# shanjiayao/PTT

Measured on AMD Instinct MI355X. Metric: tracklet frames/sec (hot path: PointNet++ SA stack + Point-Track-Transformer blocks), higher is better.
Workload: dtype f32

## Files before the change

### include/ptt_hip.h

```cpp
#ifndef PTT_HIP_H
#define PTT_HIP_H

#include <stddef.h>
#include <stdint.h>

#ifdef __cplusplus
extern "C" {
#endif

#define PTT_ABI_VERSION 25

enum {
    PTT_OK = 0,
    PTT_EINVAL = -1,
    PTT_EUNSUPPORTED = -2,
    PTT_ELAUNCH = -3,
    PTT_EWORKSPACE = -4
};

typedef void* ptt_stream_t;

int ptt_version(void);
const char* ptt_error_name(int code);
const char* ptt_last_error_string(void);

int ptt_fps_f32(const float* xyz, int B, int N, int npoint, int32_t* idx_out,
                ptt_stream_t stream);
int ptt_fps_ws_f32(const float* xyz, int B, int N, int npoint, int32_t* idx_out, float* workspace,
                   size_t workspace_elems, ptt_stream_t stream);

int ptt_gather_f32(const float* feat, const int32_t* idx, int B, int C, int N, int M,
                   float* out, ptt_stream_t stream);
int ptt_gather_grad_f32(const float* grad_out, const int32_t* idx, int B, int C, int N,
// ... 447 lines not shown
```

### ptt_amd/_lib.py

```python
import ctypes
import os
from ctypes import POINTER, Structure, c_char_p, c_double, c_float, c_int, c_int32, c_int64, c_longlong, c_size_t, c_uint32, c_void_p

_HERE = os.path.dirname(os.path.abspath(__file__))
LIB_PATH = os.path.join(_HERE, "lib", "libptt_hip.so")

PTT_SA_MAX_LAYERS = 4
ABI_VERSION = 25

EXPORTS = [
    "ptt_version", "ptt_error_name", "ptt_last_error_string",
    "ptt_fps_f32", "ptt_fps_ws_f32", "ptt_spatial_order_f32", "ptt_ball_query_grid_workspace", "ptt_ball_query_grid_f32",
    "ptt_centres_ball_query_grid_f32", "ptt_gather_f32", "ptt_gather_grad_f32", "ptt_select_centres_f32", "ptt_ball_query_f32",
    "ptt_group_f32", "ptt_group_grad_f32", "ptt_scatter_add_det_workspace", "ptt_scatter_add_det_f32",
    "ptt_knn_f32", "ptt_knn_rel_f32",
    "ptt_packed_weight_elems", "ptt_pack_weight_f32", "ptt_pack_weight_rot_f32", "ptt_linear_f32",
    "ptt_sa_fused_fwd_f32", "ptt_xcorr_fused_fwd_f32", "ptt_cosine_map_f32", "ptt_pt_attn_pair_f32",
    "ptt_crop_compact_f32", "ptt_regularize_f32", "ptt_mt19937_fill", "ptt_select_box_f32",
    "ptt_track_crop_bounds", "ptt_track_box_by_offset",
    "ptt_bn_stats_workspace", "ptt_bn_stats_f32", "ptt_bn_apply_f32", "ptt_bn_bwd_f32", "ptt_pool_rows_f32",
    "ptt_pool_rows_bwd_f32", "ptt_linear_wgrad_workspace", "ptt_linear_wgrad_f32",
    "ptt_pack_weight_strided_f32", "ptt_linear_batched_f32", "ptt_softmax_rows_f32", "ptt_layernorm_f32",
    "ptt_gather_rows_f32", "ptt_scatter_csr_i32", "ptt_scatter_rows_csr_f32",
    "ptt_pt_pair_input_f32", "ptt_pt_attn_train_fwd_f32", "ptt_pt_attn_train_bwd_f32", "ptt_linear_act_in_f32",
    "ptt_centres_ball_query_f32",
    "ptt_bn_sums_f64", "ptt_bn_finish_f64", "ptt_bn_bwd_sums_f64", "ptt_bn_bwd_apply_f32",
    "ptt_rows_mlp_f32",
    "ptt_rows_gemm_supported", "ptt_rows_gemm_stat_chunks", "ptt_rows_gemm_f32", "ptt_rows_gemm_masked_f32", "ptt_bn_finish_partials_f32",
    "ptt_bn_sums_partials_f64", "ptt_linear_wgrad2_workspace", "ptt_linear_wgrad2_f32",
    "ptt_bn_bwd_pooled_f32", "ptt_bn_bwd_pooled_sums_f64", "ptt_bn_bwd_pooled_apply_f32",
    "ptt_pt_pair_input_ld_f32", "ptt_pt_attn_fwd_ld_f32",
# ... 302 lines not shown
```

### ptt_amd/csrc/mfma_ops.hip

```cpp
#include <math.h>
#include <stdlib.h>
#include <string.h>
#include "common.h"
#include "mfma_common.h"

#ifndef PTT_PAIR_PF
#define PTT_PAIR_PF 1
#endif
#ifndef PTT_GATHER_BATCH
#define PTT_GATHER_BATCH 16
#endif
#ifndef PTT_SA_WAVES
#define PTT_SA_WAVES 2
#endif

namespace ptt {

#ifdef PTT_DEV
#define PTT_STAMP(i) do { if (p.dbg && threadIdx.x == 0 && blockIdx.x < 4096) p.dbg[blockIdx.x * 8 + (i)] = __builtin_readcyclecounter(); } while (0)
#else
#define PTT_STAMP(i) do { } while (0)
#endif

__device__ __forceinline__ void stagger_second_slot(int first_wave_blocks, int quanta) {
// ... 1243 lines not shown
                        p.out[b * p.osb + col * p.osc + mm * p.osm] = m1;
                    }
                }
            }
        }
    }
    __builtin_amdgcn_wave_barrier();
}

constexpr int SAC_HDR = 16;
struct SacTable {
    int32_t* ws; int T;
    __host__ __device__ int32_t* ndist() const { return ws + SAC_HDR; }
    __host__ __device__ int32_t* list(int k) const { return ws + SAC_HDR + (size_t)(1 + k) * T; }
    __host__ __device__ int32_t* rows(int k) const { return ws + SAC_HDR + 5 * (size_t)T + (size_t)((4 << k) - 4) * T; }
    static size_t words(size_t T) { return SAC_HDR + 65 * T; }
};
constexpr int SAC_PASSES = 4;

__global__ __launch_bounds__(64) void sa_compact_zero_kernel(int32_t* ws) {
    if (threadIdx.x < 4) ws[threadIdx.x] = 0;
}

__global__ __launch_bounds__(256) void sa_compact_kernel(const float* __restrict__ xyz, const int32_t* __restrict__ idx, int N, int M,
                                                         SacTable tab) {
    __shared__ int s_cnt[4], s_base[4], s_cls[32], s_pos[32], s_nd[32];
    __shared__ int s_row[32][32];
    const int t = threadIdx.x, lane = t & 63, half = lane >> 5, s = lane & 31, w = t >> 6;
    const int g0 = blockIdx.x * 32, T = tab.T;
    if (t < 4) s_cnt[t] = 0;
    __syncthreads();
    int iv[SAC_PASSES];
    uint32_t x[SAC_PASSES], y[SAC_PASSES], z[SAC_PASSES];
#pragma unroll
    for (int q = 0; q < SAC_PASSES; ++q) iv[q] = idx[(size_t)min(g0 + q * 8 + w * 2 + half, T - 1) * 32 + s];
#pragma unroll
    for (int q = 0; q < SAC_PASSES; ++q) {
        const int b = min(g0 + q * 8 + w * 2 + half, T - 1) / M;
        const uint32_t* pt = reinterpret_cast<const uint32_t*>(xyz) + ((size_t)b * N + iv[q]) * 3;
        x[q] = pt[0]; y[q] = pt[1]; z[q] = pt[2];
    }
#pragma unroll
    for (int q = 0; q < SAC_PASSES; ++q) {
        const int lc = q * 8 + w * 2 + half;
        const int i0a = __builtin_amdgcn_readlane(iv[q], 0), i0b = __builtin_amdgcn_readlane(iv[q], 32);
        const int i0 = half ? i0b : i0a;
        const bool real = s == 0 || iv[q] != i0;
        const unsigned long long rm = __ballot(real);
        const int J = 31 - __builtin_clz((uint32_t)rm | (uint32_t)(rm >> 32));
        int dup = 0;
        for (int j = 0; j < J; ++j) {
            const uint32_t xa = __builtin_amdgcn_readlane(x[q], j), xb = __builtin_amdgcn_readlane(x[q], 32 + j);
            const uint32_t ya = __builtin_amdgcn_readlane(y[q], j), yb = __builtin_amdgcn_readlane(y[q], 32 + j);
            const uint32_t za = __builtin_amdgcn_readlane(z[q], j), zb = __builtin_amdgcn_readlane(z[q], 32 + j);
            dup |= (int)(j < s) & (int)(x[q] == (half ? xb : xa)) & (int)(y[q] == (half ? yb : ya)) & (int)(z[q] == (half ? zb : za));
        }
        const bool keep = real && !dup;
        const unsigned long long km = __ballot(keep);
        const uint32_t m = half ? (uint32_t)(km >> 32) : (uint32_t)km;
        const int nd = __popc(m);
        if (keep) s_row[lc][__popc(m & ((1u << s) - 1u))] = iv[q];
        if (s == 0) {
            const int k = nd <= 4 ? 0 : nd <= 8 ? 1 : nd <= 16 ? 2 : 3;
            const bool valid = g0 + lc < T;
            s_cls[lc] = valid ? k : -1;
            s_nd[lc] = nd;
            s_pos[lc] = valid ? atomicAdd(&s_cnt[k], 1) : 0;
            if (valid) tab.ndist()[g0 + lc] = nd;
        }
    }
    __syncthreads();
    if (t < 4) s_base[t] = s_cnt[t] ? atomicAdd(&tab.ws[t], s_cnt[t]) : 0;
    __syncthreads();
    for (int e = t; e < 32 * 32; e += 256) {
        const int lc = e >> 5, j = e & 31, k = s_cls[lc];
        if (k < 0 || j >= (4 << k)) continue;
        const int q = s_base[k] + s_pos[lc];
        tab.rows(k)[(size_t)q * (4 << k) + j] = s_row[lc][j < s_nd[lc] ? j : 0];
        if (j == 0) tab.list(k)[q] = g0 + lc;
    }
}

#ifndef PTT_SAL_WGS
#define PTT_SAL_WGS 1
#endif
#ifndef PTT_SAL_WAVES
#define PTT_SAL_WAVES 12
#endif

struct SacTile {
    int k, first, n;
    __device__ __forceinline__ void at(int j, const int (&tiles)[4], const int (&cnt)[4]) {
        k = j < tiles[0] ? 0 : j < tiles[1] ? 1 : j < tiles[2] ? 2 : 3;
        const int j0 = k == 0 ? 0 : k == 1 ? tiles[0] : k == 2 ? tiles[1] : tiles[2];
        const int nk = k == 0 ? cnt[0] : k == 1 ? cnt[1] : k == 2 ? cnt[2] : cnt[3];
        first = (j - j0) << (3 - k);
        n = min(8 >> k, nk - first);
    }
    __device__ __forceinline__ void row(const SacTable& tab, int s, int& n_out, int& ball) const {
        const int cl = s >> (2 + k), inb = cl < n;
        n_out = tab.rows(k)[(size_t)first * (4 << k) + (inb ? s : (s & ((4 << k) - 1)))];
        ball = tab.list(k)[first + (inb ? cl : 0)];
    }
};

__device__ __forceinline__ void sac_store(const SaParams& p, const SacTile& tc, int ball, const f32x16 (&acc)[4], const float* cst,
                                          int half, int col, int osb, int osm, int osc) {
    const int k = tc.k, relu = p.L[2].relu;
    int ob[8];
#pragma unroll
    for (int g = 0; g < 8; ++g) {
        if (g >= (8 >> k)) break;
        const int id = __builtin_amdgcn_readlane(ball, g << (2 + k)), b = id / p.M;
        ob[g] = b * osb + (id - b * p.M) * osm;
    }
#pragma unroll
    for (int u = 0; u < 4; ++u) {
        const float sh = cst[(6 + u) * 64];
        float* o = p.out + (u * 32 + col) * osc;
        const f32x16& a = acc[u];
        if (k == 3) {
            const float mx = sas_pool(a, sh, relu);
            if (half == 0) o[ob[0]] = mx;
        } else if (k == 2) {
            float m0 = a[0], m1 = a[8];
#pragma unroll
            for (int r = 1; r < 8; ++r) { m0 = fmaxf(m0, a[r]); m1 = fmaxf(m1, a[8 + r]); }
            m0 = max_halves(m0) + sh; m1 = max_halves(m1) + sh;
            if (relu) { m0 = fmaxf(m0, 0.f); m1 = fmaxf(m1, 0.f); }
            if (half < tc.n) o[half ? ob[1] : ob[0]] = half ? m1 : m0;
        } else {
            float m[4];
#pragma unroll
            for (int q = 0; q < 4; ++q) m[q] = fmaxf(fmaxf(a[4 * q], a[4 * q + 1]), fmaxf(a[4 * q + 2], a[4 * q + 3]));
            if (k == 1) {
#pragma unroll
                for (int q = 0; q < 4; ++q) m[q] = max_halves(m[q]) + sh;
#pragma unroll
                for (int i = 0; i < 2; ++i) {
                    const int g = 2 * half + i;
                    float v = half ? m[2 + i] : m[i];
                    if (relu) v = fmaxf(v, 0.f);
                    if (g < tc.n) o[half ? ob[2 + i] : ob[i]] = v;
                }
            } else {
#pragma unroll
                for (int q = 0; q < 4; ++q) {
                    const int g = 2 * q + half;
                    float v = m[q] + sh;
                    if (relu) v = fmaxf(v, 0.f);
                    if (g < tc.n) o[half ? ob[2 * q + 1] : ob[2 * q]] = v;
                }
            }
        }
    }
}

template <bool COMPACT>
__global__ __launch_bounds__(64 * PTT_SAL_WAVES) __attribute__((amdgpu_waves_per_eu(PTT_SAL_WAVES * PTT_SAL_WGS / 4)))
void sa_lds_kernel(SaParams p) {
    extern __shared__ __attribute__((aligned(16))) float smem[];
    float* W1 = smem;
    float* W2 = smem + 4096;
    const int t = threadIdx.x, lane = t & 63, half = lane >> 5, col = lane & 31;
    const int w = __builtin_amdgcn_readfirstlane(t >> 6);
    const int total = p.B * p.M, M = p.M, N = p.N;
    const int nw = (int)blockDim.x >> 6;
    SacTable tab{p.cws, total};
    int cnt[4], tiles[4];
    if constexpr (COMPACT) {
#pragma unroll
        for (int k = 0; k < 4; ++k) {
            cnt[k] = min(max(p.cws[k], 0), total);
            tiles[k] = (k ? tiles[k - 1] : 0) + ((cnt[k] + (8 >> k) - 1) >> (3 - k));
        }
        if (logical_block() >= tiles[3]) return;
    }
    {
        const f32x4* g1 = reinterpret_cast<const f32x4*>(p.L[1].Wp);
        const f32x4* g2 = reinterpret_cast<const f32x4*>(p.L[2].Wp);
        f32x4* s1 = reinterpret_cast<f32x4*>(W1);
        f32x4* s2 = reinterpret_cast<f32x4*>(W2);
        const int nthr = (int)blockDim.x;
        for (int i = t; i < 1024; i += nthr) s1[i] = g1[i];
        for (int i = t; i < 2048; i += nthr) s2[i] = g2[i];
    }
    float* cst = smem + 4096 + 8192 + w * 640 + lane;
#pragma unroll
    for (int u = 0; u < 2; ++u) {
        const f32x4 f = reinterpret_cast<const f32x4*>(p.L[0].Wp)[u * 64 + col];
        const float s0 = p.L[0].shift ? p.L[0].shift[u * 32 + col] : 0.f;
        cst[(0 + u) * 64] = half ? f[1] : f[0];
        cst[(2 + u) * 64] = half ? s0 : f[2];
        cst[(4 + u) * 64] = p.L[1].shift ? p.L[1].shift[u * 32 + col] : 0.f;
    }
#pragma unroll
    for (int u = 0; u < 4; ++u) cst[(6 + u) * 64] = p.L[2].shift ? p.L[2].shift[u * 32 + col] : 0.f;
    const float one_zero = half ? 0.f : 1.f, one_hi = 1.f;
// ... 97 lines not shown
            cx = p.new_xyz[(size_t)g * 3]; cy = p.new_xyz[(size_t)g * 3 + 1]; cz = p.new_xyz[(size_t)g * 3 + 2];
        }
        __builtin_amdgcn_sched_barrier(0);
        {
            f32x16 acc[4];
#pragma unroll
            for (int kb = 0; kb < 8; ++kb) {
                if (kb < 7) {
#pragma unroll
                    for (int u = 0; u < 4; ++u) wm[u] = *reinterpret_cast<const f32x4*>(b2p + ((kb + 1) * 4 + u) * 256);
                }
                __builtin_amdgcn_sched_barrier(0);
#pragma unroll
                for (int j = 0; j < 4; ++j)
#pragma unroll
                    for (int u = 0; u < 4; ++u)
                        acc[u] = __builtin_amdgcn_mfma_f32_32x32x2f32(h1[kb >> 2][(kb & 3) * 4 + j], wb[u][j],
                                                                       (kb == 0 && j == 0) ? zero16 : acc[u], 0, 0, 0);
                __builtin_amdgcn_sched_barrier(0);
#pragma unroll
                for (int u = 0; u < 4; ++u) wb[u] = wm[u];
            }
            if constexpr (COMPACT) {
                sac_store(p, tc, g_cur, acc, cst, half, col, osb, osm, osc);
            } else {
                float* o = p.out + (ce.b * osb + ce.m * osm);
#pragma unroll
                for (int u = 0; u < 4; ++u) {
                    const float mx = sas_pool(acc[u], cst[(6 + u) * 64], p.L[2].relu);
                    if (half == 0) o[(u * 32 + col) * osc] = mx;
                }
            }
        }
        if constexpr (COMPACT) { tc = tx; g_cur = g_next; } else ce = nx;
    }
}

template <int NS, int RT>
__global__ __launch_bounds__(256, 2) void sa_wave_kernel(SaParams p) {
    extern __shared__ __attribute__((aligned(16))) float smem[];
    constexpr int CPW = 32 * RT / NS;
    const int t = threadIdx.x, lane = t & 63, w = t >> 6;
    float* Xw = smem + w * 32 * RT * p.ldk;
    const int total_centres = p.B * p.M;
    const int centre0 = (logical_block() * 4 + w) * CPW;
    if (centre0 >= total_centres) return;
    const int ncentres = min(CPW, total_centres - centre0);

#pragma unroll
    for (int rt = 0; rt < RT; ++rt) sa_gather_rows<NS, 32>(p, Xw, rt * 32, centre0, lane);
    __builtin_amdgcn_wave_barrier();

    for (int l = 0; l < p.n_layers; ++l) {
        const SaLayerDev& L = p.L[l];
        const bool last = (l == p.n_layers - 1);
#define PTT_WAVE_LAYER(CTV)                                                                         \
        { if (L.scale) sa_wave_layer<NS, CTV, true, RT>(p, L, last, Xw, lane, centre0, ncentres);       \
// ... 385 lines not shown
                    (p.fsb & 3) == 0 && (reinterpret_cast<uintptr_t>(p.feat) & 15) == 0) ? 1 : 0;
    p.first_wave = 1024; p.stagger = dev_switches().sa_stagger;
    p.dbg = dev_switches().stamps;
    p.cws = nullptr;
    const int total_centres = d->B * d->M;
    hipStream_t s = as_stream(stream);
    int rc;
    if (d->C == 0 && d->use_xyz && !hoist && d->nsample == 32 && d->n_layers == 3 && p.L[0].Cout == 64 && p.L[1].Cout == 64 &&
        p.L[2].Cout == 128 && !p.L[0].scale && !p.L[1].scale && !p.L[2].scale && p.L[0].relu && p.L[1].relu &&
        dev_switches().sa_lds) {
        const int waves = 256 * PTT_SAL_WAVES * PTT_SAL_WGS;
        p.chunk = (total_centres + waves - 1) / waves;
        if (dev_switches().sa_lds_chunk > 0 && p.chunk > dev_switches().sa_lds_chunk) p.chunk = dev_switches().sa_lds_chunk;
        const int nw = total_centres * 3 <= 256 * PTT_SAL_WAVES ? 4 : PTT_SAL_WAVES;
        int wgs = (total_centres + p.chunk * nw - 1) / (p.chunk * nw);
        const int lds = (4096 + 8192 + PTT_SAL_WAVES * 640) * (int)sizeof(float);
        if (d->compact_ws) {
            if (d->compact_ws_bytes < ptt_sa_compact_workspace(d->B, d->M) || (reinterpret_cast<uintptr_t>(d->compact_ws) & 15))
                return fail(PTT_EWORKSPACE, "ptt_sa_fused_fwd_f32: compact_ws needs %zu bytes, 16-byte aligned (got %zu)",
                            ptt_sa_compact_workspace(d->B, d->M), d->compact_ws_bytes);
            p.cws = static_cast<int32_t*>(d->compact_ws);
            hipLaunchKernelGGL(sa_compact_zero_kernel, dim3(1), dim3(64), 0, s, p.cws);
            if ((rc = check_launch("sa_compact_zero_kernel"))) return rc;
            hipLaunchKernelGGL(sa_compact_kernel, dim3((total_centres + 31) / 32), dim3(256), 0, s, d->xyz, d->idx, d->N, d->M,
                               SacTable{p.cws, total_centres});
            if ((rc = check_launch("sa_compact_kernel"))) return rc;
            if (wgs > 256 * PTT_SAL_WGS) wgs = 256 * PTT_SAL_WGS;
            if ((rc = set_lds_limit(reinterpret_cast<const void*>(sa_lds_kernel<true>), lds))) return rc;
            hipLaunchKernelGGL(sa_lds_kernel<true>, dim3(wgs), dim3(64 * nw), lds, s, p);
            return check_launch("sa_lds_kernel");
        }
        if ((rc = set_lds_limit(reinterpret_cast<const void*>(sa_lds_kernel<false>), lds))) return rc;
        hipLaunchKernelGGL(sa_lds_kernel<false>, dim3(wgs), dim3(64 * nw), lds, s, p);
        return check_launch("sa_lds_kernel");
    }
    size_t wbytes = 0;
    bool wave_ok = true;
    for (int l = 0; l < d->n_layers; ++l) {
        wbytes += (size_t)d->layers[l].Cin * d->layers[l].Cout * sizeof(float);
        const int nt = d->layers[l].Cout / 32;
        if (!(nt == 1 || nt == 2 || nt == 4)) wave_ok = false;
    }
    wave_ok = wave_ok && dev_switches().sa_wave;
    if (wave_ok && wbytes <= 64 * 1024 && d->nsample <= 32) {
        const int lds = 4 * 32 * p.ldk * (int)sizeof(float);
        const int cpw = 32 / d->nsample, per_wg = 4 * cpw;
        const dim3 grid((total_centres + per_wg - 1) / per_wg);
        if (d->nsample == 32) {
            if ((rc = set_lds_limit(reinterpret_cast<const void*>(sa_wave_kernel<32, 1>), lds))) return rc;
            hipLaunchKernelGGL((sa_wave_kernel<32, 1>), grid, dim3(256), lds, s, p);
        } else {
            if ((rc = set_lds_limit(reinterpret_cast<const void*>(sa_wave_kernel<16, 1>), lds))) return rc;
            hipLaunchKernelGGL((sa_wave_kernel<16, 1>), grid, dim3(256), lds, s, p);
        }
        return check_launch("sa_wave_kernel");
    }
    if (p.hoist == 2 && d->nsample == 32 && d->n_layers == 2 && p.L[0].Cin == 128 && p.L[0].Cout == 128 &&
        p.L[1].Cout == 256 && !p.L[0].scale && !p.L[1].scale && p.L[0].relu && dev_switches().sa_stream) {
        p.tiles = (total_centres + 1) / 2;
        int wgs = p.tiles < 512 ? p.tiles : 512;
        p.chunk = (p.tiles + wgs - 1) / wgs;
        if (dev_switches().sa_chunk > 0 && p.chunk > dev_switches().sa_chunk) p.chunk = dev_switches().sa_chunk;
        wgs = (p.tiles + p.chunk - 1) / p.chunk;
        const int lds = (2 * SAS_TILE + 4 * 16 * 4) * (int)sizeof(float);
        if ((rc = set_lds_limit(reinterpret_cast<const void*>(sa_stream_kernel<32>), lds))) return rc;
        hipLaunchKernelGGL((sa_stream_kernel<32>), dim3(wgs), dim3(256), lds, s, p);
        return check_launch("sa_stream_kernel");
    }
    int RT = dev_switches().sa_rt;
    if (d->nsample == 64) RT = 2;
    const int lds = 32 * RT * p.ldk * (int)sizeof(float);
    if (lds > 160 * 1024) return fail(PTT_EUNSUPPORTED, "ptt_sa_fused_fwd_f32: %d B of LDS per workgroup", lds);
    const int cpw = 32 * RT / d->nsample;
    const dim3 grid((total_centres + cpw - 1) / cpw);
#define PTT_SA_CASE(NSV, RTV)                                                                                   \
    if (d->nsample == NSV && RT == RTV) {                                                                       \
        if ((rc = set_lds_limit(reinterpret_cast<const void*>(sa_fused_kernel<NSV, RTV>), lds))) return rc;     \
        hipLaunchKernelGGL((sa_fused_kernel<NSV, RTV>), grid, dim3(256), lds, s, p);                            \
    }
    PTT_SA_CASE(32, 2) PTT_SA_CASE(32, 1) PTT_SA_CASE(16, 2) PTT_SA_CASE(16, 1) PTT_SA_CASE(64, 2)
#undef PTT_SA_CASE
    return check_launch("sa_fused_kernel");
}

extern "C" int ptt_xcorr_fused_fwd_f32(const ptt_xcorr_desc* d, ptt_stream_t stream) {
    if (!d) return fail(PTT_EINVAL, "ptt_xcorr_fused_fwd_f32: null descriptor");
// ... 113 lines not shown
```

### ptt_amd/models/backbones_3d/pointnet2/pointnet2_modules.py

```python
import os
from typing import List

import torch
import torch.nn as nn
import torch.nn.functional as F

from .... import ops, train_ops
from . import pointnet2_utils
from . import pytorch_utils as pt_utils


class PointnetSAModuleVotes(nn.Module):
    def __init__(self, *, mlp: List[int], radius: float = None, nsample: int = None, bn: bool = True,
                 use_xyz: bool = True, normalize_xyz: bool = False, sample_uniformly: bool = False,
                 sample_method='fps'):
        super().__init__()
        self.radius = radius
        self.nsample = nsample
        self.mlp_module = None
        self.use_xyz = use_xyz
        self.normalize_xyz = normalize_xyz
        self.sample_uniformly = sample_uniformly
        self.grouper = pointnet2_utils.QueryAndGroup(radius, nsample, use_xyz=use_xyz, ret_grouped_xyz=True,
                                                     normalize_xyz=normalize_xyz, sample_uniformly=sample_uniformly,
                                                     ret_unique_cnt=False)
        mlp_spec = mlp
        if use_xyz and len(mlp_spec) > 0:
            mlp_spec[0] += 3
        self.mlp_module = pt_utils.SharedMLP(mlp_spec, bn=bn)
        self.sample_method = sample_method
        self._fused_cache = None
        self._arange_cache = None
# ... 65 lines not shown
                if hasattr(unit, 'normlayer'):
                    bn = unit.normlayer.bn
                    scale = (bn.weight / torch.sqrt(bn.running_var + bn.eps)).float().contiguous()
                    shift = (bn.bias - bn.running_mean * scale).float().contiguous()
                    if unit.conv.bias is not None:
                        shift = (shift + unit.conv.bias * scale).contiguous()
                elif unit.conv.bias is not None:
                    shift = unit.conv.bias.detach().float().contiguous()
                wq = w if scale is None else w * scale.view(-1, 1, 1, 1)
                layers.append((ops.pack_weight(wq, rot), None, shift, cin, cout, hasattr(unit, 'activation'), scale))
            hoist = None
            w0 = self.mlp_module[0].conv.weight
            if (self.use_xyz and len(layers) >= 2 and w0.shape[1] > 3 and layers[0][4] <= 256
                    and os.environ.get('PTT_SA_HOIST', '1') != '0'):
                w2 = w0.reshape(w0.shape[0], w0.shape[1]).float()
                scale0 = layers[0][6]
                wx = w2[:, 0:3] if scale0 is None else w2[:, 0:3] * scale0[:, None]
                wf = w2[:, 3:] if scale0 is None else w2[:, 3:] * scale0[:, None]
                hoist = (ops.pack_weight(wf.contiguous()), wx.t().contiguous(), layers[0][4], layers[0][5])
        ops.publish_params(device)
        self._fused_cache = (key, (layers, hoist))
        return layers, hoist

    def forward(self, xyz: torch.Tensor, features: torch.Tensor, npoint: int, inds: torch.Tensor = None, pre=None):
        fused = self._fusable(xyz, features)
        if pre is not None and not fused:
            pre = None
        self.centres_knn = None
        if (fused and pre is None and inds is None and self.sample_method == 'fps' and xyz.shape[1] <= 256 and npoint <= 128
                and xyz.shape[0] * npoint * self.nsample <= ops.ONE_FRAME_MAX_SA_ROWS and self.centres_knn_k <= npoint):
            xyz = xyz.contiguous()
            inds, inds64, new_xyz, idx, self.centres_knn = ops.fps_ball_knn(xyz, npoint, self.radius, self.nsample, self.centres_knn_k)
            pre = (new_xyz, idx, inds64)
        prefix = inds is None and self.sample_method in ('rs', 'sequence')
        if pre is not None:
            pass
        elif fused and prefix:
            key = (xyz.size(0), npoint, str(xyz.device))
            if self._arange_cache is None:
                self._arange_cache = {}
            if key not in self._arange_cache:
                self._arange_cache[key] = torch.arange(npoint, dtype=torch.int64, device=xyz.device).repeat(
                    xyz.size(0), 1)
                ops.publish_params(xyz.device, replaced=False)
            inds64 = self._arange_cache[key]
        elif inds is None:
            inds = self._sample(xyz, features, npoint)
# ... 7 lines not shown
                new_xyz, idx, inds64 = pre
            elif prefix:
                new_xyz, _, idx = ops.centres_ball_query(xyz, None, npoint, self.radius, self.nsample)
            else:
                new_xyz, inds64, idx = ops.centres_ball_query(xyz, inds.contiguous(), npoint, self.radius, self.nsample)
            layers, hoist = self._fused_params(xyz.device)
            if hoist is not None and features is not None:
                wf_packed, wx, c0, relu0 = hoist
                rows = features.transpose(1, 2)
                uniform = rows.stride(2) == 1 and rows.stride(0) == rows.shape[1] * rows.stride(1)
                term = ops.linear(rows if uniform else rows.contiguous(), wf_packed, c0, None, layers[0][2], relu=False)
                B, M, ns = xyz.shape[0], npoint, self.nsample
                if (B * M * ns <= ops.ONE_FRAME_MAX_SA_ROWS and ns in (16, 32) and len(layers) == 3 and c0 % 4 == 0 and c0 >= 192):
                    L1, L2 = layers[1], layers[2]
                    h = torch.empty((B * M * ns, L1[4]), dtype=torch.float32, device=xyz.device)
                    ops.row_jobs([ops.row_job(L1[0], L1[4], prologue=3, x=term, idx=idx, xyz=xyz, centres=new_xyz, wx=wx,
                                              radius=self.radius, ns=ns, M=M, N=xyz.shape[1], normalize_xyz=self.normalize_xyz,
                                              pro_relu=relu0, scale=L1[1], shift=L1[2], act=1 if L1[5] else 0, out=h)])
                    pooled = torch.empty((B, M, L2[4]), dtype=torch.float32, device=xyz.device)
                    ops.row_jobs([ops.row_job(L2[0], L2[4], x=h, epilogue=2, ns=ns, M=M, scale=L2[1], shift=L2[2],
                                              act=1 if L2[5] else 0, out=pooled)])
                    return new_xyz, pooled.transpose(1, 2), inds64
                new_features = ops.sa_fused_forward(xyz, new_xyz, idx, None, [L[:6] for L in layers[1:]], self.radius, True,
                                                    self.normalize_xyz, point_major_out=True, l0=(term, wx, relu0))
            else:
                new_features = ops.sa_fused_forward(xyz, new_xyz, idx, features, [L[:6] for L in layers], self.radius,
                                                    self.use_xyz, self.normalize_xyz, point_major_out=True,
                                                    compact=features is None)
            return new_xyz, new_features, inds64

        hoist = (self.use_xyz and not self.sample_uniformly and self.nsample * npoint <= 16384
                 and train_ops.usable(self.mlp_module, xyz if features is None else features)
                 and self.mlp_module[0].conv.weight.shape[0] % 4 == 0)
        if hoist and not xyz.requires_grad and inds.dtype == torch.int32:
            new_xyz, inds64, idx = ops.centres_ball_query(xyz.contiguous(), inds.contiguous(), npoint, self.radius, self.nsample)
            y = train_ops.sa_level_hoisted(xyz, new_xyz, features, idx, self.mlp_module, self.radius, self.normalize_xyz)
            return new_xyz, y, inds64
        xyz_flipped = xyz.transpose(1, 2).contiguous()
        new_xyz = pointnet2_utils.gather_operation(xyz_flipped, inds).transpose(1, 2).contiguous()
        if hoist and features is not None:
            idx = pointnet2_utils.ball_query(self.radius, self.nsample, xyz, new_xyz)
            y = train_ops.sa_level_hoisted(xyz, new_xyz, features, idx, self.mlp_module, self.radius, self.normalize_xyz)
            return new_xyz, y, inds.to(torch.int64)
        grouped_features, grouped_xyz = self.grouper(xyz, new_xyz, features)
        if train_ops.usable(self.mlp_module, grouped_features):
            return new_xyz, train_ops.shared_mlp_pool(grouped_features, self.mlp_module, pool_dim=3), inds.to(torch.int64)
        y = self.mlp_module(grouped_features)
# ... 3 lines not shown
```

### ptt_amd/models/backbones_3d/pointnet2_backbone.py

```python
from typing import List

import torch
import torch.nn as nn

from ... import graph_policy, ops, train_ops
from .pointnet2 import pointnet2_modules


class PointNet2BackboneLight(nn.Module):
    def __init__(self, model_cfg, input_channels, **kwargs):
        super().__init__()
        self.model_cfg = model_cfg
        input_channels -= 3
        self.num_points_each_layer = []
        self.SA_modules = nn.ModuleList()
        sa = self.model_cfg.SA_CONFIG
        for k in range(len(sa.RADIUS)):
            mlps = list(sa.MLPS[k])
            if k == 0:
                mlps[0] = input_channels
            self.SA_modules.append(pointnet2_modules.PointnetSAModuleVotes(
                radius=sa.RADIUS[k], nsample=sa.NSAMPLE[k], mlp=mlps,
                use_xyz=sa.get('USE_XYZ', True), normalize_xyz=sa.get('NORMALIZE_XYZ', True),
                sample_method=sa.SAMPLE_METHOD[k]))
# ... 17 lines not shown
            if features.dtype != torch.float32:
                return self.cov_final(features)
            return train_ops.rows_linear(self.cov_final, features.transpose(1, 2)).transpose(1, 2)
        if ops.autograd_recording(self.cov_final, features) or features.dtype != torch.float32:
            ops.note_unfused('PointNet2BackboneLight.cov_final', 'autograd is recording or input is not float32')
            return self.cov_final(features)
        w, b = self.cov_final.weight, self.cov_final.bias
        key = (w.data_ptr(), w._version, b.data_ptr(), b._version)
        if self._cov_cache is None or self._cov_cache[0] != key:
            self._cov_cache = (key, ops.pack_weight(w), b.detach().float().contiguous())
            ops.publish_params(w.device)
        rows = features.transpose(1, 2)
        out = ops.linear(rows, self._cov_cache[1], w.shape[0], None, self._cov_cache[2])
        return out.transpose(1, 2)

    def _arange64(self, xyz, n):
        key = (xyz.size(0), n, str(xyz.device))
        cache = self.__dict__.setdefault('_arange_cache', {})
        if key not in cache:
            cache[key] = torch.arange(n, dtype=torch.int64, device=xyz.device).repeat(xyz.size(0), 1)
            ops.publish_params(xyz.device, replaced=False)
        return cache[key]

    def branch_forward(self, pts, npoints: List, inds0=None, want_knn=0):
        xyz, features = self._break_up_pc(pts)
        sa = self.model_cfg.SA_CONFIG
        one_frame = (not self.training and xyz.is_cuda and features is None and len(self.SA_modules) == 3
                     and xyz.shape[0] * npoints[0] <= 4 * ops.ONE_FRAME_MAX_POINTS
                     and self.SA_modules[0].sample_method == 'fps'
                     and all(m.sample_method in ('rs', 'sequence') for m in self.SA_modules[1:])
                     and npoints[0] >= npoints[1] >= npoints[2] and (not want_knn or npoints[2] <= 128)
                     and all(m._fusable(xyz, None) for m in self.SA_modules[:1]))
        knn = None
        if one_frame:
            from .pointnet2 import pointnet2_utils
            xyz = xyz.contiguous()
            if inds0 is None:
                inds0 = pointnet2_utils.furthest_point_sample(xyz, npoints[0])
            inds0 = inds0.to(torch.int32).contiguous()
            levels, inds64, knn = ops.sa_levels_point_jobs(xyz, inds0, list(npoints), list(sa.RADIUS), list(sa.NSAMPLE),
                                                           knn_k=want_knn)
            seq = [None, self._arange64(xyz, npoints[1]), self._arange64(xyz, npoints[2])]
            xyz, features, inds0 = self.SA_modules[0](xyz=xyz, features=features, npoint=npoints[0], inds=inds0,
                                                      pre=(levels[0][0], levels[0][1], inds64))
            xyz, features, inds1 = self.SA_modules[1](xyz=xyz, features=features, npoint=npoints[1],
                                                      pre=(levels[1][0], levels[1][1], seq[1]))
            xyz, features, inds2 = self.SA_modules[2](xyz=xyz, features=features, npoint=npoints[2],
                                                      pre=(levels[2][0], levels[2][1], seq[2]))
        else:
            xyz, features, inds0 = self.SA_modules[0](xyz=xyz, features=features, npoint=npoints[0], inds=inds0)
            xyz, features, inds1 = self.SA_modules[1](xyz=xyz, features=features, npoint=npoints[1])
            xyz, features, inds2 = self.SA_modules[2](xyz=xyz, features=features, npoint=npoints[2])
        point_features = self._cov_final(features)
        assert inds1.dtype == inds2.dtype == torch.int64, 'index type must be int64, not {}'.format(inds2.dtype)
        if all(m.sample_method in ('rs', 'sequence') for m in self.SA_modules[1:]) and inds0.shape[1] >= npoints[2]:
            inds = inds0[:, :npoints[2]]
        else:
            inds = inds0.gather(1, inds1).gather(1, inds2)
        if want_knn:
            return xyz, point_features, inds, knn
        return xyz, point_features, inds

    def sample(self, search_points, template_points):
        from .pointnet2 import pointnet2_utils
        sa = self.model_cfg.SA_CONFIG
        assert sa.SAMPLE_METHOD[0] == 'fps'
        return (pointnet2_utils.furthest_point_sample(search_points[..., 0:3].contiguous(), sa.NPOINTS_SEARCH[0]),
                pointnet2_utils.furthest_point_sample(template_points[..., 0:3].contiguous(), sa.NPOINTS_TEMPLATE[0]))

    def forward_branches(self, search_points, template_points, inds=None):
        sa = self.model_cfg.SA_CONFIG
        i_s, i_t = inds if inds is not None else (None, None)
        if not (self.overlap_branches and search_points.is_cuda and not self.training):
            r = self.branch_forward(search_points, sa.NPOINTS_SEARCH, i_s, want_knn=self.seed_knn)
            t_seeds, t_feats, t_inds = self.branch_forward(template_points, sa.NPOINTS_TEMPLATE, i_t)
        else:
            if self._side_stream is None or self._side_stream.device != search_points.device:
                self._side_stream = torch.cuda.Stream(device=search_points.device)
            main = torch.cuda.current_stream(search_points.device)
            side = graph_policy.branch(main, self._side_stream)
            with torch.cuda.stream(side):
                t_seeds, t_feats, t_inds = self.branch_forward(template_points, sa.NPOINTS_TEMPLATE, i_t)
            r = self.branch_forward(search_points, sa.NPOINTS_SEARCH, i_s, want_knn=self.seed_knn)
            graph_policy.join(main, side)
            if side is not main:
                for t in (t_seeds, t_feats, t_inds, template_points):
                    t.record_stream(main)
        s_seeds, s_feats, s_inds = r[:3]
        s_knn = r[3] if len(r) > 3 else None
        out = {'search_seeds': s_seeds, 'search_feats': s_feats, 'search_inds': s_inds,
               'template_seeds': t_seeds, 'template_feats': t_feats, 'template_inds': t_inds}
        if s_knn is not None:
            out['search_seeds_knn'] = s_knn
        return out

    def forward(self, batch_dict):
        batch_dict.update(self.forward_branches(batch_dict['search_points'], batch_dict['template_points'],
                                                batch_dict.pop('fps_inds', None)))
        batch_dict.pop('search_points')
        batch_dict.pop('template_points')
        return batch_dict
```

Measured before the change: 16750.

## Add compacted streaming SA kernel for last search-branch level

Adds a new sa_stream_compact_kernel that processes balls grouped by distinct-neighbour count in 64-row tiles, so the two MLP layers and max-pool run only on unique neighbour rows. It also adds an XYZ-free variant of the compaction pre-pass that dedups by index only, skipping the coordinate comparison. The path is enabled for the last SA level of the search branch in inference when there are many balls and few input points. This adds an extra compaction launch and a separate code path, and its benefit depends on how many duplicate neighbours the ball query produces.

```diff
diff --git a/include/ptt_hip.h b/include/ptt_hip.h
--- a/include/ptt_hip.h
+++ b/include/ptt_hip.h
@@ -8,7 +8,7 @@
 extern "C" {
 #endif
 
-#define PTT_ABI_VERSION 25
+#define PTT_ABI_VERSION 26
 
 enum {
     PTT_OK = 0,
diff --git a/ptt_amd/_lib.py b/ptt_amd/_lib.py
--- a/ptt_amd/_lib.py
+++ b/ptt_amd/_lib.py
@@ -6,7 +6,7 @@
 LIB_PATH = os.path.join(_HERE, "lib", "libptt_hip.so")
 
 PTT_SA_MAX_LAYERS = 4
-ABI_VERSION = 25
+ABI_VERSION = 26
 
 EXPORTS = [
     "ptt_version", "ptt_error_name", "ptt_last_error_string",
diff --git a/ptt_amd/csrc/mfma_ops.hip b/ptt_amd/csrc/mfma_ops.hip
--- a/ptt_amd/csrc/mfma_ops.hip
+++ b/ptt_amd/csrc/mfma_ops.hip
@@ -1289,6 +1289,7 @@
     if (threadIdx.x < 4) ws[threadIdx.x] = 0;
 }
 
+template <bool XYZ>
 __global__ __launch_bounds__(256) void sa_compact_kernel(const float* __restrict__ xyz, const int32_t* __restrict__ idx, int N, int M,
                                                          SacTable tab) {
     __shared__ int s_cnt[4], s_base[4], s_cls[32], s_pos[32], s_nd[32];
@@ -1301,11 +1302,13 @@
     uint32_t x[SAC_PASSES], y[SAC_PASSES], z[SAC_PASSES];
 #pragma unroll
     for (int q = 0; q < SAC_PASSES; ++q) iv[q] = idx[(size_t)min(g0 + q * 8 + w * 2 + half, T - 1) * 32 + s];
-#pragma unroll
-    for (int q = 0; q < SAC_PASSES; ++q) {
-        const int b = min(g0 + q * 8 + w * 2 + half, T - 1) / M;
-        const uint32_t* pt = reinterpret_cast<const uint32_t*>(xyz) + ((size_t)b * N + iv[q]) * 3;
-        x[q] = pt[0]; y[q] = pt[1]; z[q] = pt[2];
+    if constexpr (XYZ) {
+#pragma unroll
+        for (int q = 0; q < SAC_PASSES; ++q) {
+            const int b = min(g0 + q * 8 + w * 2 + half, T - 1) / M;
+            const uint32_t* pt = reinterpret_cast<const uint32_t*>(xyz) + ((size_t)b * N + iv[q]) * 3;
+            x[q] = pt[0]; y[q] = pt[1]; z[q] = pt[2];
+        }
     }
 #pragma unroll
     for (int q = 0; q < SAC_PASSES; ++q) {
@@ -1313,14 +1316,16 @@
         const int i0a = __builtin_amdgcn_readlane(iv[q], 0), i0b = __builtin_amdgcn_readlane(iv[q], 32);
         const int i0 = half ? i0b : i0a;
         const bool real = s == 0 || iv[q] != i0;
-        const unsigned long long rm = __ballot(real);
-        const int J = 31 - __builtin_clz((uint32_t)rm | (uint32_t)(rm >> 32));
         int dup = 0;
-        for (int j = 0; j < J; ++j) {
-            const uint32_t xa = __builtin_amdgcn_readlane(x[q], j), xb = __builtin_amdgcn_readlane(x[q], 32 + j);
-            const uint32_t ya = __builtin_amdgcn_readlane(y[q], j), yb = __builtin_amdgcn_readlane(y[q], 32 + j);
-            const uint32_t za = __builtin_amdgcn_readlane(z[q], j), zb = __builtin_amdgcn_readlane(z[q], 32 + j);
-            dup |= (int)(j < s) & (int)(x[q] == (half ? xb : xa)) & (int)(y[q] == (half ? yb : ya)) & (int)(z[q] == (half ? zb : za));
+        if constexpr (XYZ) {
+            const unsigned long long rm = __ballot(real);
+            const int J = 31 - __builtin_clz((uint32_t)rm | (uint32_t)(rm >> 32));
+            for (int j = 0; j < J; ++j) {
+                const uint32_t xa = __builtin_amdgcn_readlane(x[q], j), xb = __builtin_amdgcn_readlane(x[q], 32 + j);
+                const uint32_t ya = __builtin_amdgcn_readlane(y[q], j), yb = __builtin_amdgcn_readlane(y[q], 32 + j);
+                const uint32_t za = __builtin_amdgcn_readlane(z[q], j), zb = __builtin_amdgcn_readlane(z[q], 32 + j);
+                dup |= (int)(j < s) & (int)(x[q] == (half ? xb : xa)) & (int)(y[q] == (half ? yb : ya)) & (int)(z[q] == (half ? zb : za));
+            }
         }
         const bool keep = real && !dup;
         const unsigned long long km = __ballot(keep);
@@ -1355,14 +1360,24 @@
 #define PTT_SAL_WAVES 12
 #endif
 
-struct SacTile {
+template <int ROWS>
+struct SacTileT {
+    static constexpr int LG = ROWS == 32 ? 3 : 4;
+    static_assert(ROWS == 32 || ROWS == 64, "32- or 64-row tiles");
     int k, first, n;
+    __device__ __forceinline__ static void count(const int32_t* ws, int total, int (&cnt)[4], int (&tiles)[4]) {
+#pragma unroll
+        for (int k = 0; k < 4; ++k) {
+            cnt[k] = min(max(ws[k], 0), total);
+            tiles[k] = (k ? tiles[k - 1] : 0) + ((cnt[k] + ((1 << LG) >> k) - 1) >> (LG - k));
+        }
+    }
     __device__ __forceinline__ void at(int j, const int (&tiles)[4], const int (&cnt)[4]) {
         k = j < tiles[0] ? 0 : j < tiles[1] ? 1 : j < tiles[2] ? 2 : 3;
         const int j0 = k == 0 ? 0 : k == 1 ? tiles[0] : k == 2 ? tiles[1] : tiles[2];
         const int nk = k == 0 ? cnt[0] : k == 1 ? cnt[1] : k == 2 ? cnt[2] : cnt[3];
-        first = (j - j0) << (3 - k);
-        n = min(8 >> k, nk - first);
+        first = (j - j0) << (LG - k);
+        n = min((1 << LG) >> k, nk - first);
     }
     __device__ __forceinline__ void row(const SacTable& tab, int s, int& n_out, int& ball) const {
         const int cl = s >> (2 + k), inb = cl < n;
@@ -1370,53 +1385,52 @@
         ball = tab.list(k)[first + (inb ? cl : 0)];
     }
 };
-
-__device__ __forceinline__ void sac_store(const SaParams& p, const SacTile& tc, int ball, const f32x16 (&acc)[4], const float* cst,
-                                          int half, int col, int osb, int osm, int osc) {
-    const int k = tc.k, relu = p.L[2].relu;
+using SacTile = SacTileT<32>;
+
+template <int NU>
+__device__ __forceinline__ void sac_store(int k, int n, int ball, int M, const f32x16 (&acc)[NU], const float (&sh)[NU],
+                                          float* const (&o)[NU], int relu, int half, int osb, int osm) {
     int ob[8];
 #pragma unroll
     for (int g = 0; g < 8; ++g) {
         if (g >= (8 >> k)) break;
-        const int id = __builtin_amdgcn_readlane(ball, g << (2 + k)), b = id / p.M;
-        ob[g] = b * osb + (id - b * p.M) * osm;
-    }
-#pragma unroll
-    for (int u = 0; u < 4; ++u) {
-        const float sh = cst[(6 + u) * 64];
-        float* o = p.out + (u * 32 + col) * osc;
+        const int id = __builtin_amdgcn_readlane(ball, g << (2 + k)), b = id / M;
+        ob[g] = b * osb + (id - b * M) * osm;
+    }
+#pragma unroll
+    for (int u = 0; u < NU; ++u) {
         const f32x16& a = acc[u];
         if (k == 3) {
-            const float mx = sas_pool(a, sh, relu);
-            if (half == 0) o[ob[0]] = mx;
+            const float mx = sas_pool(a, sh[u], relu);
+            if (half == 0) o[u][ob[0]] = mx;
         } else if (k == 2) {
             float m0 = a[0], m1 = a[8];
 #pragma unroll
             for (int r = 1; r < 8; ++r) { m0 = fmaxf(m0, a[r]); m1 = fmaxf(m1, a[8 + r]); }
-            m0 = max_halves(m0) + sh; m1 = max_halves(m1) + sh;
+            m0 = max_halves(m0) + sh[u]; m1 = max_halves(m1) + sh[u];
             if (relu) { m0 = fmaxf(m0, 0.f); m1 = fmaxf(m1, 0.f); }
-            if (half < tc.n) o[half ? ob[1] : ob[0]] = half ? m1 : m0;
+            if (half < n) o[u][half ? ob[1] : ob[0]] = half ? m1 : m0;
         } else {
             float m[4];
 #pragma unroll
             for (int q = 0; q < 4; ++q) m[q] = fmaxf(fmaxf(a[4 * q], a[4 * q + 1]), fmaxf(a[4 * q + 2], a[4 * q + 3]));
             if (k == 1) {
 #pragma unroll
-                for (int q = 0; q < 4; ++q) m[q] = max_halves(m[q]) + sh;
+                for (int q = 0; q < 4; ++q) m[q] = max_halves(m[q]) + sh[u];
 #pragma unroll
                 for (int i = 0; i < 2; ++i) {
                     const int g = 2 * half + i;
                     float v = half ? m[2 + i] : m[i];
                     if (relu) v = fmaxf(v, 0.f);
-                    if (g < tc.n) o[half ? ob[2 + i] : ob[i]] = v;
+                    if (g < n) o[u][half ? ob[2 + i] : ob[i]] = v;
                 }
             } else {
 #pragma unroll
                 for (int q = 0; q < 4; ++q) {
                     const int g = 2 * q + half;
-                    float v = m[q] + sh;
+                    float v = m[q] + sh[u];
                     if (relu) v = fmaxf(v, 0.f);
-                    if (g < tc.n) o[half ? ob[2 * q + 1] : ob[2 * q]] = v;
+                    if (g < n) o[u][half ? ob[2 * q + 1] : ob[2 * q]] = v;
                 }
             }
         }
@@ -1436,11 +1450,7 @@
     SacTable tab{p.cws, total};
     int cnt[4], tiles[4];
     if constexpr (COMPACT) {
-#pragma unroll
-        for (int k = 0; k < 4; ++k) {
-            cnt[k] = min(max(p.cws[k], 0), total);
-            tiles[k] = (k ? tiles[k - 1] : 0) + ((cnt[k] + (8 >> k) - 1) >> (3 - k));
-        }
+        SacTile::count(p.cws, total, cnt, tiles);
         if (logical_block() >= tiles[3]) return;
     }
     {
@@ -1584,7 +1594,9 @@
                 for (int u = 0; u < 4; ++u) wb[u] = wm[u];
             }
             if constexpr (COMPACT) {
-                sac_store(p, tc, g_cur, acc, cst, half, col, osb, osm, osc);
+                const float sh2[4] = {cst[6 * 64], cst[7 * 64], cst[8 * 64], cst[9 * 64]};
+                float* const o[4] = {p.out + col * osc, p.out + (32 + col) * osc, p.out + (64 + col) * osc, p.out + (96 + col) * osc};
+                sac_store<4>(tc.k, tc.n, g_cur, M, acc, sh2, o, p.L[2].relu, half, osb, osm);
             } else {
                 float* o = p.out + (ce.b * osb + ce.m * osm);
 #pragma unroll
@@ -1595,6 +1607,101 @@
             }
         }
         if constexpr (COMPACT) { tc = tx; g_cur = g_next; } else ce = nx;
+    }
+}
+
+__global__ __launch_bounds__(256, 2) void sa_stream_compact_kernel(SaParams p) {
+    extern __shared__ __attribute__((aligned(16))) float smem[];
+    float* const P = smem;
+    float* const Q = smem + SAS_TILE;
+    float* const meta = smem + 2 * SAS_TILE;
+    int* const sball = reinterpret_cast<int*>(meta + 64 * 4);
+    const int t = threadIdx.x, lane = t & 63, half = lane >> 5, sub = half, q = lane & 31, col = q;
+    const int w = __builtin_amdgcn_readfirstlane(t >> 6);
+    const int total = p.B * p.M, M = p.M, N = p.N;
+    const SacTable tab{p.cws, total};
+    int cnt[4], tiles[4];
+    SacTileT<64>::count(p.cws, total, cnt, tiles);
+    if ((int)blockIdx.x >= tiles[3]) return;
+    const SaLayerDev& L1 = p.L[0];
+    const SaLayerDev& L2 = p.L[1];
+    const __amdgpu_buffer_rsrc_t rf = weight_rsrc(p.feat);
+    const __amdgpu_buffer_rsrc_t wr1 = weight_rsrc(L1.Wp), wr2 = weight_rsrc(L2.Wp);
+    const int wvoff = (w * 64 + lane) * 16;
+    constexpr int WK1 = 4 * 1024, WK2 = 8 * 1024;
+    const f32x4 wx0 = *reinterpret_cast<const f32x4*>(p.wx + q * 4);
+    const f32x4 wx1 = *reinterpret_cast<const f32x4*>(p.wx + 128 + q * 4);
+    const f32x4 wx2 = *reinterpret_cast<const f32x4*>(p.wx + 256 + q * 4);
+    const float sh1 = L1.shift ? L1.shift[w * 32 + col] : 0.f;
+    const float sh2[2] = {L2.shift ? L2.shift[w * 32 + col] : 0.f, L2.shift ? L2.shift[(w + 4) * 32 + col] : 0.f};
+    f32x16 sh1v;
+#pragma unroll
+    for (int r = 0; r < 16; ++r) sh1v[r] = sh1;
+    const f32x16 zero16 = {0.f, 0.f, 0.f, 0.f, 0.f, 0.f, 0.f, 0.f, 0.f, 0.f, 0.f, 0.f, 0.f, 0.f, 0.f, 0.f};
+    const float floor0 = p.l0_relu ? 0.f : -__builtin_inff();
+    const float rdiv = p.normalize ? p.radius : 1.0f;
+    const int osb = (int)p.osb, osm = (int)p.osm;
+    float* const o[2] = {p.out + (w * 32 + col) * (int)p.osc, p.out + ((w + 4) * 32 + col) * (int)p.osc};
+
+    for (int j = blockIdx.x; j < tiles[3]; j += (int)gridDim.x) {
+        SacTileT<64> tc;
+        tc.at(j, tiles, cnt);
+        if (t < 64) {
+            int n, ball;
+            tc.row(tab, t, n, ball);
+            const int flat = (ball / M) * N + n;
+            const float x = p.xyz[(size_t)flat * 3 + 0], y = p.xyz[(size_t)flat * 3 + 1], z = p.xyz[(size_t)flat * 3 + 2];
+            const float cx = p.new_xyz[(size_t)ball * 3 + 0], cy = p.new_xyz[(size_t)ball * 3 + 1], cz = p.new_xyz[(size_t)ball * 3 + 2];
+            const float dx = (x - cx) / rdiv, dy = (y - cy) / rdiv, dz = (z - cz) / rdiv;
+            const int off = flat * (128 * (int)sizeof(float));
+            *reinterpret_cast<f32x4*>(meta + t * 4) = f32x4{__builtin_bit_cast(float, off), dx, dy, dz};
+            sball[t] = ball;
+        }
+        __syncthreads();
+#pragma unroll
+        for (int i = 0; i < 8; ++i) {
+            f32x4 m;
+            const f32x4 v = sas_pair_load(meta, rf, w, i, sub, q, m);
+            sas_pair_store(P, w, i, sub, q, v, m, wx0, wx1, wx2, floor0);
+        }
+        const int ballr[2] = {sball[col], sball[32 + col]};
+        __syncthreads();
+        {
+            f32x16 acc1[2] = {sh1v, sh1v};
+            const float* arow = P + (lane & 31) * SAS_LDK + 4 * half;
+#pragma unroll
+            for (int kb = 0; kb < 16; ++kb) {
+                const f32x4 b = weight_load(wr1, wvoff, kb * WK1);
+                const f32x4 a[2] = {*reinterpret_cast<const f32x4*>(arow + kb * 8),
+                                    *reinterpret_cast<const f32x4*>(arow + 32 * SAS_LDK + kb * 8)};
+#pragma unroll
+                for (int jj = 0; jj < 4; ++jj)
+#pragma unroll
+                    for (int rt = 0; rt < 2; ++rt) acc1[rt] = __builtin_amdgcn_mfma_f32_32x32x2f32(a[rt][jj], b[jj], acc1[rt], 0, 0, 0);
+            }
+#pragma unroll
+            for (int rt = 0; rt < 2; ++rt)
+#pragma unroll
+                for (int r = 0; r < 16; ++r) Q[(rt * 32 + tile_row(r, half)) * SAS_LDK + w * 32 + col] = fmaxf(acc1[rt][r], 0.f);
+        }
+        __syncthreads();
+        {
+            f32x16 acc[2][2] = {{zero16, zero16}, {zero16, zero16}};
+            const float* arow = Q + (lane & 31) * SAS_LDK + 4 * half;
+#pragma unroll
+            for (int kb = 0; kb < 16; ++kb) {
+                const f32x4 b[2] = {weight_load(wr2, wvoff, kb * WK2), weight_load(wr2, wvoff, kb * WK2 + 4 * 1024)};
+                const f32x4 a[2] = {*reinterpret_cast<const f32x4*>(arow + kb * 8),
+                                    *reinterpret_cast<const f32x4*>(arow + 32 * SAS_LDK + kb * 8)};
+                gemm_mfma_block<2, 2, 2>(a, b, acc);
+            }
+#pragma unroll
+            for (int rt = 0; rt < 2; ++rt) {
+                const int n = tc.n - rt * (8 >> tc.k);
+                if (n <= 0) continue;
+                sac_store<2>(tc.k, n, ballr[rt], M, acc[rt], sh2, o, L2.relu, half, osb, osm);
+            }
+        }
     }
 }
 
@@ -2026,7 +2133,7 @@
             p.cws = static_cast<int32_t*>(d->compact_ws);
             hipLaunchKernelGGL(sa_compact_zero_kernel, dim3(1), dim3(64), 0, s, p.cws);
             if ((rc = check_launch("sa_compact_zero_kernel"))) return rc;
-            hipLaunchKernelGGL(sa_compact_kernel, dim3((total_centres + 31) / 32), dim3(256), 0, s, d->xyz, d->idx, d->N, d->M,
+            hipLaunchKernelGGL(sa_compact_kernel<true>, dim3((total_centres + 31) / 32), dim3(256), 0, s, d->xyz, d->idx, d->N, d->M,
                                SacTable{p.cws, total_centres});
             if ((rc = check_launch("sa_compact_kernel"))) return rc;
             if (wgs > 256 * PTT_SAL_WGS) wgs = 256 * PTT_SAL_WGS;
@@ -2066,6 +2173,21 @@
         p.chunk = (p.tiles + wgs - 1) / wgs;
         if (dev_switches().sa_chunk > 0 && p.chunk > dev_switches().sa_chunk) p.chunk = dev_switches().sa_chunk;
         wgs = (p.tiles + p.chunk - 1) / p.chunk;
+        if (d->compact_ws) {
+            if (d->compact_ws_bytes < ptt_sa_compact_workspace(d->B, d->M) || (reinterpret_cast<uintptr_t>(d->compact_ws) & 15))
+                return fail(PTT_EWORKSPACE, "ptt_sa_fused_fwd_f32: compact_ws needs %zu bytes, 16-byte aligned (got %zu)",
+                            ptt_sa_compact_workspace(d->B, d->M), d->compact_ws_bytes);
+            p.cws = static_cast<int32_t*>(d->compact_ws);
+            hipLaunchKernelGGL(sa_compact_zero_kernel, dim3(1), dim3(64), 0, s, p.cws);
+            if ((rc = check_launch("sa_compact_zero_kernel"))) return rc;
+            hipLaunchKernelGGL(sa_compact_kernel<false>, dim3((total_centres + 31) / 32), dim3(256), 0, s, d->xyz, d->idx, d->N, d->M,
+                               SacTable{p.cws, total_centres});
+            if ((rc = check_launch("sa_compact_kernel"))) return rc;
+            const int lds = (2 * SAS_TILE + 64 * 4 + 64) * (int)sizeof(float);
+            if ((rc = set_lds_limit(reinterpret_cast<const void*>(sa_stream_compact_kernel), lds))) return rc;
+            hipLaunchKernelGGL(sa_stream_compact_kernel, dim3(p.tiles < 512 ? p.tiles : 512), dim3(256), lds, s, p);
+            return check_launch("sa_stream_compact_kernel");
+        }
         const int lds = (2 * SAS_TILE + 4 * 16 * 4) * (int)sizeof(float);
         if ((rc = set_lds_limit(reinterpret_cast<const void*>(sa_stream_kernel<32>), lds))) return rc;
         hipLaunchKernelGGL((sa_stream_kernel<32>), dim3(wgs), dim3(256), lds, s, p);
diff --git a/ptt_amd/models/backbones_3d/pointnet2/pointnet2_modules.py b/ptt_amd/models/backbones_3d/pointnet2/pointnet2_modules.py
--- a/ptt_amd/models/backbones_3d/pointnet2/pointnet2_modules.py
+++ b/ptt_amd/models/backbones_3d/pointnet2/pointnet2_modules.py
@@ -8,6 +8,9 @@
 from .... import ops, train_ops
 from . import pointnet2_utils
 from . import pytorch_utils as pt_utils
+
+STREAM_COMPACT_MIN_BALLS = 2048
+STREAM_COMPACT_MAX_POINTS = 1024
 
 
 class PointnetSAModuleVotes(nn.Module):
@@ -119,7 +122,8 @@
         self._fused_cache = (key, (layers, hoist))
         return layers, hoist
 
-    def forward(self, xyz: torch.Tensor, features: torch.Tensor, npoint: int, inds: torch.Tensor = None, pre=None):
+    def forward(self, xyz: torch.Tensor, features: torch.Tensor, npoint: int, inds: torch.Tensor = None, pre=None,
+                compact: bool = False):
         fused = self._fusable(xyz, features)
         if pre is not None and not fused:
             pre = None
@@ -173,7 +177,9 @@
                                               act=1 if L2[5] else 0, out=pooled)])
                     return new_xyz, pooled.transpose(1, 2), inds64
                 new_features = ops.sa_fused_forward(xyz, new_xyz, idx, None, [L[:6] for L in layers[1:]], self.radius, True,
-                                                    self.normalize_xyz, point_major_out=True, l0=(term, wx, relu0))
+                                                    self.normalize_xyz, point_major_out=True, l0=(term, wx, relu0),
+                                                    compact=(bool(compact) and B * M >= STREAM_COMPACT_MIN_BALLS
+                                                             and xyz.shape[1] <= STREAM_COMPACT_MAX_POINTS))
             else:
                 new_features = ops.sa_fused_forward(xyz, new_xyz, idx, features, [L[:6] for L in layers], self.radius,
                                                     self.use_xyz, self.normalize_xyz, point_major_out=True,
diff --git a/ptt_amd/models/backbones_3d/pointnet2_backbone.py b/ptt_amd/models/backbones_3d/pointnet2_backbone.py
--- a/ptt_amd/models/backbones_3d/pointnet2_backbone.py
+++ b/ptt_amd/models/backbones_3d/pointnet2_backbone.py
@@ -63,7 +63,7 @@
             ops.publish_params(xyz.device, replaced=False)
         return cache[key]
 
-    def branch_forward(self, pts, npoints: List, inds0=None, want_knn=0):
+    def branch_forward(self, pts, npoints: List, inds0=None, want_knn=0, compact_levels=()):
         xyz, features = self._break_up_pc(pts)
         sa = self.model_cfg.SA_CONFIG
         one_frame = (not self.training and xyz.is_cuda and features is None and len(self.SA_modules) == 3
@@ -90,8 +90,8 @@
                                                       pre=(levels[2][0], levels[2][1], seq[2]))
         else:
             xyz, features, inds0 = self.SA_modules[0](xyz=xyz, features=features, npoint=npoints[0], inds=inds0)
-            xyz, features, inds1 = self.SA_modules[1](xyz=xyz, features=features, npoint=npoints[1])
-            xyz, features, inds2 = self.SA_modules[2](xyz=xyz, features=features, npoint=npoints[2])
+            xyz, features, inds1 = self.SA_modules[1](xyz=xyz, features=features, npoint=npoints[1], compact=1 in compact_levels)
+            xyz, features, inds2 = self.SA_modules[2](xyz=xyz, features=features, npoint=npoints[2], compact=2 in compact_levels)
         point_features = self._cov_final(features)
         assert inds1.dtype == inds2.dtype == torch.int64, 'index type must be int64, not {}'.format(inds2.dtype)
         if all(m.sample_method in ('rs', 'sequence') for m in self.SA_modules[1:]) and inds0.shape[1] >= npoints[2]:
@@ -112,8 +112,9 @@
     def forward_branches(self, search_points, template_points, inds=None):
         sa = self.model_cfg.SA_CONFIG
         i_s, i_t = inds if inds is not None else (None, None)
+        last = (len(self.SA_modules) - 1,) if (search_points.is_cuda and not self.training) else ()
         if not (self.overlap_branches and search_points.is_cuda and not self.training):
-            r = self.branch_forward(search_points, sa.NPOINTS_SEARCH, i_s, want_knn=self.seed_knn)
+            r = self.branch_forward(search_points, sa.NPOINTS_SEARCH, i_s, want_knn=self.seed_knn, compact_levels=last)
             t_seeds, t_feats, t_inds = self.branch_forward(template_points, sa.NPOINTS_TEMPLATE, i_t)
         else:
             if self._side_stream is None or self._side_stream.device != search_points.device:
@@ -122,7 +123,7 @@
             side = graph_policy.branch(main, self._side_stream)
             with torch.cuda.stream(side):
                 t_seeds, t_feats, t_inds = self.branch_forward(template_points, sa.NPOINTS_TEMPLATE, i_t)
-            r = self.branch_forward(search_points, sa.NPOINTS_SEARCH, i_s, want_knn=self.seed_knn)
+            r = self.branch_forward(search_points, sa.NPOINTS_SEARCH, i_s, want_knn=self.seed_knn, compact_levels=last)
             graph_policy.join(main, side)
             if side is not main:
                 for t in (t_seeds, t_feats, t_inds, template_points):
```

After: 17410 (median of 6 runs). 1.04x the previous value.
